# swiss-territorial-data-lab/proj-roadsurf

Measured on AMD Instinct MI355X. Metric: tiles_per_sec_512x512x3, higher is better.
Workload: dtype f16 hi + lo operand planes (22 significand bits, 3 MFMA products per product) / f32 accumulate; 1 GPU; Mask R-CNN R50-FPN inference, batch 16 of 512x512 3-band tiles per GPU (BASELINE configs[1]), 800x800 network input; seeded synthetic weights, saturated: 1000 proposals and 100 detections per tile; batch_per_gpu=16, lanes=2, lane_streams=independent, num_classes=2, weights=random

## Files before the change

### proj_roadsurf_amd/csrc/conv_wide1x1_split.hip

```cpp
#include "conv_tile.h"

namespace {

constexpr int PR = 32;
constexpr int KS = 8;
constexpr int SLICE = KS * PR * 128;
constexpr int LDS_BYTES = 2 * SLICE;

__device__ __forceinline__ float dot_term(float s, float v, float w, bool fused) {
  if (fused) return __builtin_fmaf(v, w, s);
  {
#pragma clang fp contract(off)
    const float m = v * w;
    return s + m;
  }
}

template <int NW, int NJ, int MODE>
__global__ __launch_bounds__(NW * 64, NW == 4 ? 2 : 1) void conv_wide1x1_split_kernel(const ConvParams p) {
  constexpr int BM = NW * NJ * 16;
  constexpr int NG = 32 / NW;
  constexpr int ST = MODE == 2 ? NJ : 4 * NJ;
  extern __shared__ __attribute__((aligned(16))) char smem[];
  const int tid = threadIdx.x, lane = tid & 63;
  const int wave = __builtin_amdgcn_readfirstlane(tid >> 6);
  const int M = conv_rows(p);
  const int ntiles = (M + BM - 1) / BM;
  const int q = blockIdx.x;
  if (q >= ntiles) return;
  const int m0 = xcd_tile(q, ntiles) * BM;
  const int rows = p.Cout * (MODE == 2 ? 4 : 1);
  const int npass = rows / PR;

  const int lrow = lane >> 3, lchk = lane & 7;
  const int rp = wave & 3, s0 = wave >> 2;
  const half_t* wsrc;
  {
    const int d = src_chunk(lchk, w_key(8 * rp + lrow, 8));
    wsrc = p.w + (long long)(rp * 16 + lrow) * p.Kpad + s0 * 32 + chunk_split(d, p.w_lo);
  }
  auto stage_piece = [&](int pass, int k) {
    const half_t* g = wsrc + (long long)((pass >> 1) * 64 + (pass & 1) * 8) * p.Kpad;
    char* base = smem + (pass & 1) * SLICE + (s0 * PR + rp * 8) * 128;
    glds16(g + k * (NW / 4) * 32, base + k * (NW / 4) * PR * 128);
  };

  const int fi = lane & 15, fq = lane >> 4, fkey = lane & 7;
  int w_off[2];
#pragma unroll
  for (int ii = 0; ii < 2; ++ii) w_off[ii] = frag_row(fi, ii, 8) * 128;
  const int ch_off = frag_off(fq, fkey, 0), cl_off = frag_off(fq, fkey, 1);

  half8 xh[KS][NJ], xl[KS][NJ];
  bool valid[NJ];
  long long opix[NJ];
  const float* wv[NJ];
  const bool full = m0 + (wave + 1) * NJ * 16 <= M;
#pragma unroll
  for (int j = 0; j < NJ; ++j) {
    const int m = m0 + (wave * NJ + j) * 16 + fi;
    valid[j] = m < M;
    const int mm = valid[j] ? m : M - 1;
    const Pix px = pix_of(mm, p.Wo, p.Ho);
    const int x = px.x, y = px.y, n = px.n;
    const half_t* xp = p.in + ((long long)(n * p.in_Hp + y + p.in_off) * p.in_Wp + x + p.in_off) * 256 + fq * 8;
#pragma unroll
    for (int s = 0; s < KS; ++s) { xh[s][j] = *(const half8*)(xp + s * 32); xl[s][j] = *(const half8*)(xp + p.in_lo + s * 32); }
    if (MODE == 2) {
      const int slot = p.dot_slot[n];
      wv[j] = p.dot_w + (long long)p.dot_cls[slot] * p.Cout;
      opix[j] = (long long)slot * (4 * p.Ho * p.Wo) + (long long)(2 * y) * (2 * p.Wo) + 2 * x;
    } else {
      wv[j] = nullptr;
      opix[j] = (long long)(n * p.out_Hp + y + p.out_pad) * p.out_Wp + x + p.out_pad;
    }
  }
  const bool has_res = MODE == 0 && p.res != nullptr;
  half8 rh[NJ], rl[NJ], qh[NJ], ql[NJ];
  auto load_res = [&](int pass, half8* h, half8* l) {
    const int c = (pass >> 1) * 64 + fq * 16 + (pass & 1) * 8;
#pragma unroll
    for (int j = 0; j < NJ; ++j) {
      const half_t* rp2 = p.res + opix[j] * p.out_Cs + c;
      h[j] = *(const half8*)rp2;
      l[j] = *(const half8*)(rp2 + p.res_lo);
    }
  };
#pragma unroll
  for (int j = 0; j < NJ; ++j) { rh[j] = half8{0, 0, 0, 0, 0, 0, 0, 0}; rl[j] = rh[j]; qh[j] = rh[j]; ql[j] = rh[j]; }
#pragma unroll
  for (int k = 0; k < NG; ++k) stage_piece(0, k);
  if (has_res) load_res(0, rh, rl);

#pragma unroll
  for (int s = 0; s < KS; ++s)
#pragma unroll
    for (int j = 0; j < NJ; ++j) asm volatile("" ::"v"(xh[s][j]), "v"(xl[s][j]));
  float sdot[NJ], gsum[NJ];
  half8 kh[MODE == 0 ? NJ : 1], kl[MODE == 0 ? NJ : 1];
#pragma unroll
  for (int j = 0; j < NJ; ++j) { sdot[j] = 0.f; gsum[j] = 0.f; }
  int pend = 0;
  auto run_pass = [&](const int pass, half8 (&ch)[NJ], half8 (&cl)[NJ], half8 (&nh)[NJ], half8 (&nl)[NJ]) __attribute__((always_inline)) {
    if (pend) asm volatile("s_waitcnt vmcnt(%0)" ::"n"(ST) : "memory");
    else asm volatile("s_waitcnt vmcnt(0)" ::: "memory");
    asm volatile("s_waitcnt lgkmcnt(0)" ::: "memory");
    __builtin_amdgcn_s_barrier();
    const bool more = pass + 1 < npass;
    if (more && has_res) load_res(pass + 1, nh, nl);
    const int crow = (pass >> 1) * 64 + fq * 16 + (pass & 1) * 8;
    const int g = MODE == 2 ? crow / p.Cout : 0, cb = crow - g * p.Cout;
    float bias[8], wsc[8];
    float dw[MODE == 2 ? NJ : 1][8];
    auto load_epi = [&]() {
#pragma unroll
      for (int ii = 0; ii < 2; ++ii) {
        const f32x4 b4 = *(const f32x4*)(p.bias + crow + ii * 4), s4 = *(const f32x4*)(p.wscale + crow + ii * 4);
#pragma unroll
        for (int r = 0; r < 4; ++r) { bias[ii * 4 + r] = b4[r]; wsc[ii * 4 + r] = s4[r]; }
      }
      if (MODE == 2) {
#pragma unroll
        for (int j = 0; j < NJ; ++j)
#pragma unroll
          for (int ii = 0; ii < 2; ++ii) {
            const f32x4 w4 = *(const f32x4*)(wv[j] + cb + ii * 4);
#pragma unroll
            for (int r = 0; r < 4; ++r) dw[j][ii * 4 + r] = w4[r];
          }
      }
    };
    __builtin_amdgcn_sched_barrier(0);
    const char* sb = smem + (pass & 1) * SLICE;
    f32x4 acc[2][NJ];
#pragma unroll
    for (int ii = 0; ii < 2; ++ii)
#pragma unroll
      for (int j = 0; j < NJ; ++j) acc[ii][j] = f32x4{0.f, 0.f, 0.f, 0.f};
    auto frag = [&](int s, int ii, int off) { return *(const half8*)(sb + s * (PR * 128) + w_off[ii] + off); };
    half8 wh[2], wl[2], nwh[2];
#pragma unroll
    for (int ii = 0; ii < 2; ++ii) { wh[ii] = frag(0, ii, ch_off); wl[ii] = frag(0, ii, cl_off); }
#pragma unroll
    for (int s = 0; s < KS; ++s) {
      if (s + 1 < KS) {
#pragma unroll
        for (int ii = 0; ii < 2; ++ii) nwh[ii] = frag(s + 1, ii, ch_off);
      }
      if (s == KS - 2) load_epi();
      if (more && 2 * s < NG) { stage_piece(pass + 1, 2 * s); stage_piece(pass + 1, 2 * s + 1); }
      __builtin_amdgcn_sched_barrier(0);
#pragma unroll
      for (int ii = 0; ii < 2; ++ii)
#pragma unroll
        for (int j = 0; j < NJ; ++j) acc[ii][j] = __builtin_amdgcn_mfma_f32_16x16x32_f16(wh[ii], xl[s][j], acc[ii][j], 0, 0, 0);
#pragma unroll
      for (int ii = 0; ii < 2; ++ii)
#pragma unroll
        for (int j = 0; j < NJ; ++j) acc[ii][j] = __builtin_amdgcn_mfma_f32_16x16x32_f16(wh[ii], xh[s][j], acc[ii][j], 0, 0, 0);
      __builtin_amdgcn_sched_barrier(0);
#pragma unroll
      for (int ii = 0; ii < 2; ++ii)
#pragma unroll
        for (int j = 0; j < NJ; ++j) acc[ii][j] = __builtin_amdgcn_mfma_f32_16x16x32_f16(wl[ii], xh[s][j], acc[ii][j], 0, 0, 0);
      __builtin_amdgcn_sched_barrier(0);
      if (s + 1 < KS) {
#pragma unroll
        for (int ii = 0; ii < 2; ++ii) { wl[ii] = frag(s + 1, ii, cl_off); wh[ii] = nwh[ii]; }
      }
    }

    if (MODE == 2) {
#pragma unroll
      for (int j = 0; j < NJ; ++j) {
        float v[8];
#pragma unroll
        for (int ii = 0; ii < 2; ++ii)
#pragma unroll
          for (int r = 0; r < 4; ++r) v[ii * 4 + r] = acc[ii][j][r] * wsc[ii * 4 + r] + bias[ii * 4 + r];
        if (p.relu) {
#pragma unroll
          for (int e = 0; e < 8; ++e) v[e] = v[e] > 0.f ? v[e] : 0.f;
        }
        float sd = sdot[j];
#pragma unroll
        for (int e = 0; e < 8; ++e) sd = dot_term(sd, v[e], dw[j][e], (pass & 1) == 0 && e < 4);
        sdot[j] = sd;
      }
      pend = 0;
      if (pass & 1) {
        const int blocks = p.Cout >> 6, k = (pass >> 1) % blocks;
#pragma unroll
        for (int j = 0; j < NJ; ++j) {
          float v0 = sdot[j];
          v0 += __shfl_xor(v0, 16);
          v0 += __shfl_xor(v0, 32);
          gsum[j] = k == 0 ? v0 : gsum[j] + v0;
          sdot[j] = 0.f;
        }
        if (k == blocks - 1) {
#pragma unroll
          for (int j = 0; j < NJ; ++j)
            if (fq == 0 && valid[j]) p.dot_out[opix[j] + (long long)(g >> 1) * (2 * p.Wo) + (g & 1)] = gsum[j];
          pend = full ? ST : 0;
        }
      }
    } else {
#pragma unroll
      for (int j = 0; j < NJ; ++j) {
        float v[8];
#pragma unroll
        for (int ii = 0; ii < 2; ++ii)
#pragma unroll
          for (int r = 0; r < 4; ++r) v[ii * 4 + r] = acc[ii][j][r] * wsc[ii * 4 + r] + bias[ii * 4 + r];
        if (has_res) {
#pragma unroll
          for (int e = 0; e < 8; ++e) v[e] += (float)ch[j][e] + (float)cl[j][e];
        }
        if (p.relu) {
#pragma unroll
          for (int e = 0; e < 8; ++e) v[e] = v[e] > 0.f ? v[e] : 0.f;
        }
        float scr = 0.f;
        half8 h, l;
#pragma unroll
        for (int e = 0; e < 8; ++e) {
          const float f = clamp_h16(v[e]);
          scr += __builtin_fabsf(f);
          const HiLo hl = split_round(f);
          h[e] = hl.h;
          l[e] = hl.l;
        }
        if (valid[j] && !(scr < 65504.f)) {
          unsigned c = 0;
#pragma unroll
          for (int e = 0; e < 8; ++e) c += rs_sat_bad(v[e]);
          rs_sat_flush(p.sat, c);
        }
        if ((pass & 1) == 0) {
          kh[j] = h; kl[j] = l;
        } else if (valid[j]) {
          half_t* op = (half_t*)p.out + opix[j] * p.out_Cs + crow - 8;
          *(half8*)op = kh[j];
          *(half8*)(op + 8) = h;
          *(half8*)(op + p.out_lo) = kl[j];
          *(half8*)(op + p.out_lo + 8) = l;
        }
      }
      pend = (pass & 1) && full ? ST : 0;
    }
  };
  for (int pass = 0; pass < npass; pass += 2) {
    run_pass(pass, rh, rl, qh, ql);
    run_pass(pass + 1, qh, ql, rh, rl);
  }
}

template <int NW, int NJ>
int launch_px(const ConvParams& p, hipStream_t stream) {
  const long long nblk = cdiv(p.M, NW * NJ * 16);
  RS_CHECK(nblk > 0 && nblk < (1ll << 31), RS_ERR_ARG, "conv_wide1x1_split: bad grid %lld", nblk);
  const void* k = p.mode == 2 ? (const void*)conv_wide1x1_split_kernel<NW, NJ, 2> : (const void*)conv_wide1x1_split_kernel<NW, NJ, 0>;
  static bool attr[2] = {false, false};
  const int ai = p.mode == 2 ? 1 : 0;
  if (!attr[ai]) {
    RS_HIP(hipFuncSetAttribute(k, hipFuncAttributeMaxDynamicSharedMemorySize, LDS_BYTES));
    attr[ai] = true;
  }
  ConvParams pc = p;
  void* args[] = {&pc};
  RS_HIP(hipLaunchKernel(k, dim3((unsigned)nblk), dim3(NW * 64), args, LDS_BYTES, stream));
  return RS_OK;
}

}

bool conv_wide1x1_split_ok(const ConvParams& p) {
  const int rows = p.Cout * (p.mode != 0 ? 4 : 1);
  return p.split && p.KH == 1 && p.KW == 1 && p.stride == 1 && p.Cin == 256 && p.in_Cs == 256 && p.Kpad >= 256 && !p.in2 && !p.up && !p.out_f32 &&
         !p.koff && !p.head_w && p.nseg == 0 && !p.down && !p.res32 && !p.mask && p.out_stride <= 1 && rows > 0 && rows % 64 == 0 &&
         (p.mode == 0 || (p.mode == 2 && p.Cout == 256)) &&
         p.Kpad % 8 == 0 && p.in_lo % 8 == 0 && p.w_lo % 8 == 0 &&
         (p.mode != 0 || (p.out_Cs % 8 == 0 && p.out_Cs >= rows && p.out_lo % 8 == 0 && p.res_lo % 8 == 0));
}

int launch_conv_wide1x1_split(const ConvParams& p, hipStream_t stream, int tile_px) {
  RS_CHECK(conv_wide1x1_split_ok(p), RS_ERR_UNSUPPORTED, "conv_wide1x1_split: takes split-operand 1x1 / stride 1 / Cin 256 layers with rows %% 64 == 0 (mode 0, or mode 2 with Cout 256)");
  RS_CHECK(p.M > 0 && p.in && p.w && p.bias && p.wscale && (!p.m_count || p.m_mul > 0), RS_ERR_ARG, "conv_wide1x1_split: null argument");
  if (p.mode == 2) RS_CHECK(p.dot_w && p.dot_cls && p.dot_slot && p.dot_out, RS_ERR_ARG, "conv_wide1x1_split: the fused mask predictor needs its pointers");
  else RS_CHECK(p.out, RS_ERR_ARG, "conv_wide1x1_split: null output");
  switch (tile_px) {
    case 64: return launch_px<4, 1>(p, stream);
    case 128: return launch_px<4, 2>(p, stream);
    case 256: return launch_px<8, 2>(p, stream);
    default: rs_set_error("conv_wide1x1_split: tile of %d pixels (64, 128 or 256)", tile_px); return RS_ERR_ARG;
  }
}
```

### proj_roadsurf_amd/csrc/ops.hip

```cpp
#include <string.h>

#include <vector>

#include "../../include/rs_engine.h"
#include "detect.h"
#include "polygon_pool.h"
#include "train.h"
#include "train_stats.h"
#include "val_ap.h"

namespace {

struct OpScratch {
  hipStream_t stream;
  void* held[2] = {nullptr, nullptr};
  int n = 0;
  explicit OpScratch(void* s) : stream((hipStream_t)s) {}
  OpScratch(const OpScratch&) = delete;
  OpScratch& operator=(const OpScratch&) = delete;
  int alloc(void** p, size_t bytes) {
    RS_CHECK(n < 2, RS_ERR_ARG, "OpScratch: more than two buffers");
    RS_HIP(hipMalloc(p, bytes));
    held[n++] = *p;
    return RS_OK;
  }
  hipError_t sync() const { return n ? hipStreamSynchronize(stream) : hipSuccess; }
  ~OpScratch() {
    (void)sync();
    for (int i = 0; i < n; ++i) (void)hipFree(held[i]);
  }
};

}

extern "C" {

__global__ void fdiv_kernel(const float* a, const float* b, float* out, long long n) {
  const long long i = (long long)blockIdx.x * 256 + threadIdx.x;
  if (i < n) out[i] = rs_fdiv(a[i], b[i]);
}
int rs_op_fdiv(const float* a, const float* b, float* out, int64_t n, void* stream) {
  RS_CHECK(a && b && out && n > 0, RS_ERR_ARG, "bad argument");
  hipLaunchKernelGGL(fdiv_kernel, dim3((unsigned)((n + 255) / 256)), dim3(256), 0, (hipStream_t)stream, a, b, out, (long long)n);
  RS_HIP(hipGetLastError());
  return RS_OK;
}

int rs_memcpy_d2h(void* dst, const void* src, size_t n) {
  RS_HIP(hipMemcpy(dst, src, n, hipMemcpyDeviceToHost));
  return RS_OK;
}
int rs_memcpy_h2d(void* dst, const void* src, size_t n) {
  RS_HIP(hipMemcpy(dst, src, n, hipMemcpyHostToDevice));
  return RS_OK;
}

int rs_op_conv_variant(int m, int cin, int k, int cout, int cin2, int deconv2x, int out_f32, int* stages_out) {
  ConvParams p;
  memset(&p, 0, sizeof p);
  p.M = m; p.Cin = cin; p.KH = p.KW = k; p.Cout = cout; p.mode = deconv2x ? 1 : 0; p.out_f32 = out_f32;
  p.stride = 1; p.in_Cs = cin; p.out_Cs = cout;
  p.Kpad = (k * k * (cin < 64 ? 8 : cin) + cin2 + 63) / 64 * 64;
  if (cin < 64 && k == 7) p.Kpad = 256;
  static const half_t dummy = (half_t)0;
  if (cin2 > 0) { p.in2 = &dummy; p.Cin2 = cin2; }
  const int v = conv_choose_variant(p, -1, 1);
  if (stages_out) *stages_out = p.stages;
  return cin < 64 ? 5 : v;
}

int rs_op_conv_variant_split(int m, int cin, int k, int stride, int cout, int cin2, int deconv_predict, int* stages_out) {
  ConvParams p;
  memset(&p, 0, sizeof p);
  p.M = m; p.Cin = cin; p.KH = p.KW = k; p.Cout = cout; p.mode = deconv_predict ? 2 : 0;
  p.stride = stride; p.in_Cs = cin; p.out_Cs = cout; p.split = 1;
  p.Kpad = (k * k * (cin < 64 ? 8 : cin) + cin2 + 63) / 64 * 64;
  if (cin < 64 && k == 7) p.Kpad = 256;
  static const half_t dummy = (half_t)0;
  if (cin2 > 0) { p.in2 = &dummy; p.Cin2 = cin2; }
  const int v = conv_choose_variant(p, -1, 1);
  if (stages_out) *stages_out = p.stages;
  return cin < 64 ? 5 : v;
}

static long long* g_conv_probe = nullptr;
static thread_local unsigned long long* g_op_sat = nullptr;
struct SplitArgs { long long in_lo, w_lo, out_lo, res_lo, up_lo; const float* wscale; };
static int op_conv2d(const void* in, const void* w, const float* bias, void* out, const void* residual, const void* upsample_add,
                     int n, int hi, int wi, int cin, int in_halo, int kh, int kw, int stride, int pad, int cout, int kpad,
                     int out_halo, int relu, int out_f32, int deconv2x, int variant, int use_glds, void* stream,
                     const void* in2, int h2, int w2, int cin2, int in2_halo, int stride2, const SplitArgs* sa = nullptr) {
  RS_CHECK(in && w && bias && out, RS_ERR_ARG, "null argument");
  RS_CHECK(in_halo >= pad, RS_ERR_ARG, "input halo %d < pad %d", in_halo, pad);
  const int ho = (hi + 2 * pad - kh) / stride + 1, wo = (wi + 2 * pad - kw) / stride + 1;
  ConvParams p;
  memset(&p, 0, sizeof p);
  p.in = (const half_t*)in; p.w = (const half_t*)w; p.bias = bias; p.out = out;
  p.res = (const half_t*)residual; p.up = (const half_t*)upsample_add;
  p.M = n * ho * wo; p.Ho = ho; p.Wo = wo;
  p.in_Hp = hi + 2 * in_halo; p.in_Wp = wi + 2 * in_halo; p.in_Cs = cin; p.in_off = in_halo - pad;
  p.stride = stride; p.KH = kh; p.KW = kw; p.Cin = cin; p.Kpad = kpad; p.Cout = cout;
  const int oh = deconv2x ? 2 * ho : ho, ow = deconv2x ? 2 * wo : wo;
  p.out_Hp = oh + 2 * out_halo; p.out_Wp = ow + 2 * out_halo; p.out_Cs = cout; p.out_pad = out_halo;
  if (upsample_add) { p.up_Hp = ho / 2 + 2 * out_halo; p.up_Wp = wo / 2 + 2 * out_halo; p.up_Cs = cout; p.up_pad = out_halo; }
  p.relu = relu; p.mode = deconv2x ? 1 : 0; p.out_f32 = out_f32;
  p.probe = g_conv_probe;
  p.sat = g_op_sat;
  if (sa) {
    RS_CHECK(sa->wscale && !in2, RS_ERR_ARG, "split-operand conv: row scales missing (or a second K source, which the operator does not take)");
    p.split = 1; p.in_lo = sa->in_lo; p.w_lo = sa->w_lo; p.out_lo = sa->out_lo; p.res_lo = sa->res_lo; p.up_lo = sa->up_lo; p.wscale = sa->wscale;
  }
  if (in2) {
    RS_CHECK(stride2 >= 1 && (ho - 1) * stride2 < h2 && (wo - 1) * stride2 < w2, RS_ERR_ARG, "second source geometry");
    p.in2 = (const half_t*)in2; p.in2_Hp = h2 + 2 * in2_halo; p.in2_Wp = w2 + 2 * in2_halo; p.in2_Cs = cin2;
    p.in2_off = in2_halo; p.stride2 = stride2; p.Cin2 = cin2;
  }
  OpScratch scratch(stream);
  if (cin < 64 && use_glds >= 0) {
    RS_CHECK(cin == 8, RS_ERR_UNSUPPORTED, "small-Cin path needs cin == 8");
    std::vector<int> koff(kpad / 8, 0);
    for (int t = 0; t < kh * kw && t < (int)koff.size(); ++t) koff[t] = ((t / kw) * p.in_Wp + (t % kw)) * cin;
    int* koff_dev = nullptr;
    { int rc = scratch.alloc((void**)&koff_dev, koff.size() * 4); if (rc) return rc; }
    RS_HIP(hipMemcpy(koff_dev, koff.data(), koff.size() * 4, hipMemcpyHostToDevice));
    p.koff = koff_dev;
  }
  return launch_conv(p, (hipStream_t)stream, variant, use_glds);
}

int rs_debug_set_conv_probe(void* buffer) { g_conv_probe = (long long*)buffer; return RS_OK; }
int rs_op_set_saturation_counter(void* dev_u64) { g_op_sat = (unsigned long long*)dev_u64; return RS_OK; }

int rs_op_conv2d(const void* in, const void* w, const float* bias, void* out, const void* residual, const void* upsample_add,
                 int n, int hi, int wi, int cin, int in_halo, int kh, int kw, int stride, int pad, int cout, int kpad,
                 int out_halo, int relu, int out_f32, int deconv2x, int variant, int use_glds, void* stream) {
  return op_conv2d(in, w, bias, out, residual, upsample_add, n, hi, wi, cin, in_halo, kh, kw, stride, pad, cout, kpad, out_halo,
                   relu, out_f32, deconv2x, variant, use_glds, stream, nullptr, 0, 0, 0, 0, 1);
}

int rs_op_conv2d_split(const void* in, int64_t in_lo, const void* w, int64_t w_lo, const float* wscale, const float* bias, void* out, int64_t out_lo,
                       const void* residual, int64_t res_lo, const void* upsample_add, int64_t up_lo,
                       int n, int hi, int wi, int cin, int in_halo, int kh, int kw, int stride, int pad, int cout, int kpad,
                       int out_halo, int relu, int out_f32, int deconv2x, int variant, void* stream) {
  SplitArgs sa = {in_lo, w_lo, out_lo, res_lo, up_lo, wscale};
  return op_conv2d(in, w, bias, out, residual, upsample_add, n, hi, wi, cin, in_halo, kh, kw, stride, pad, cout, kpad, out_halo,
                   relu, out_f32, deconv2x, variant, 1, stream, nullptr, 0, 0, 0, 0, 1, &sa);
}

int rs_op_deconv_predict_split(const void* in, int64_t in_lo, const void* w, int64_t w_lo, const float* wscale, const float* bias, const float* dot_w, int classes,
                               const int32_t* cls, const int32_t* slot, const int32_t* count_dev, float* logits, int entries, int side, int variant, void* stream) {
  RS_CHECK(in && w && wscale && bias && dot_w && cls && slot && logits && entries > 0 && side > 0 && classes > 0, RS_ERR_ARG, "deconv_predict_split: bad argument");
  ConvParams p;
  memset(&p, 0, sizeof p);
  p.in = (const half_t*)in; p.w = (const half_t*)w; p.bias = bias; p.wscale = wscale;
  p.split = 1; p.in_lo = in_lo; p.w_lo = w_lo;
  p.M = entries * side * side; p.Ho = side; p.Wo = side;
  p.in_Hp = side + 2; p.in_Wp = side + 2; p.in_Cs = 256; p.in_off = 1; p.stride = 1; p.KH = p.KW = 1; p.Cin = 256; p.Kpad = 256; p.Cout = 256;
  p.out_Hp = 2 * side; p.out_Wp = 2 * side; p.out_Cs = 256; p.relu = 1; p.mode = 2;
  p.m_count = count_dev; p.m_mul = side * side;
  p.dot_w = dot_w; p.dot_cls = cls; p.dot_slot = slot; p.dot_out = logits; p.dot_k = classes;
  return launch_conv(p, (hipStream_t)stream, variant, 1);
}

int rs_op_conv2d_dual(const void* in, const void* in2, const void* w, const float* bias, void* out,
                      int n, int hi, int wi, int cin, int in_halo, int kh, int kw, int stride, int pad,
                      int h2, int w2, int cin2, int in2_halo, int stride2,
                      int cout, int kpad, int out_halo, int relu, int variant, void* stream) {
  RS_CHECK(in2, RS_ERR_ARG, "null argument");
  return op_conv2d(in, w, bias, out, nullptr, nullptr, n, hi, wi, cin, in_halo, kh, kw, stride, pad, cout, kpad, out_halo,
                   relu, 0, 0, variant, 1, stream, in2, h2, w2, cin2, in2_halo, stride2);
}

int rs_op_bneck_tail(const void* t1, const void* w2, const float* b2, const void* w3p, const float* b3, const void* x, void* out,
                     const void* w1p, const float* b1, void* t1n, const void* x0, const void* wsc, int n, int h, int w, int width, void* stream) {
  RS_CHECK(t1 && w2 && b2 && w3p && b3 && out && n > 0 && h > 0 && w > 0, RS_ERR_ARG, "bad argument");
  RS_CHECK(width == 64 || width == 128, RS_ERR_UNSUPPORTED, "bneck_tail: bottleneck width %d (64 or 128)", width);
  BneckParams p;
  memset(&p, 0, sizeof p);
  p.t1 = (const half_t*)t1; p.w2 = (const half_t*)w2; p.b2 = b2; p.w3p = (const half_t*)w3p; p.b3 = b3; p.x = (const half_t*)x; p.out = (half_t*)out;
  p.w1p = (const half_t*)w1p; p.b1 = b1; p.t1n = (half_t*)t1n; p.x0 = (const half_t*)x0; p.wsc = (const half_t*)wsc;
  p.M = n * h * w; p.H = h; p.W = w; p.Hp = h + 2; p.Wp = w + 2; p.CB = width / 64;
  p.sat = g_op_sat;
  return launch_bneck_tail(p, (hipStream_t)stream);
}

int rs_op_bneck_tail_split(const void* t1, int64_t t1_lo, const void* w2, const float* s2, const float* b2, const void* w3p, const float* s3, const float* b3,
                           const void* x, int64_t x_lo, void* out, int64_t out_lo, const void* w1p, const float* s1, const float* b1, void* t1n, int64_t t1n_lo,
                           const void* x0, int64_t x0_lo, int n, int h, int w, int width, void* stream) {
  RS_CHECK(t1 && w2 && s2 && b2 && w3p && s3 && b3 && (x || x0) && out && n > 0 && h > 0 && w > 0, RS_ERR_ARG, "bad argument");
  RS_CHECK(width == 64 || width == 128, RS_ERR_UNSUPPORTED, "bneck_tail_split: bottleneck width %d (64 or 128)", width);
  BneckSplitParams p;
  memset(&p, 0, sizeof p);
  p.t1 = (const half_t*)t1; p.t1_lo = t1_lo;
  p.w2 = (const half_t*)w2; p.w2_lo = (long long)width * 9 * width; p.s2 = s2; p.b2 = b2;
  p.w3p = (const half_t*)w3p; p.w3_lo = 4ll * width * (width + (x0 ? 64 : 0)); p.s3 = s3; p.b3 = b3;
  p.x = (const half_t*)x; p.x_lo = x_lo; p.x0 = (const half_t*)x0; p.x0_lo = x0_lo; p.out = (half_t*)out; p.out_lo = out_lo;
  p.w1p = (const half_t*)w1p; p.w1_lo = 4ll * width * width; p.s1 = s1; p.b1 = b1; p.t1n = (half_t*)t1n; p.t1n_lo = t1n_lo;
  p.M = n * h * w; p.H = h; p.W = w; p.Hp = h + 2; p.Wp = w + 2; p.CB = width / 64;
  p.sat = g_op_sat;
  return launch_bneck_tail_split(p, (hipStream_t)stream);
}

int rs_op_mask_overlap(const uint8_t* det_masks, int n_det, const uint8_t* label_masks, int n_labels, int h, int w, int32_t* inter,
                       int32_t* label_area, void* stream) {
  return launch_mask_overlap(det_masks, n_det, label_masks, n_labels, h, w, inter, label_area, (hipStream_t)stream);
}


int rs_op_rasterize_canvas(const double* polys, const int64_t* poly_off, const int32_t* poly_len, const int32_t* inst_first, int n_inst,
                           int side, uint8_t* out) {
  RS_CHECK(inst_first && n_inst >= 0 && (out || n_inst == 0), RS_ERR_ARG, "rasterize_canvas: null table");
  RS_CHECK(side >= 1 && side <= CR_MAX_SIDE, RS_ERR_ARG, "rasterize_canvas: side %d outside [1, %d]", side, CR_MAX_SIDE);
  MtLayout L;
  { int rc = mt_measure(polys, poly_off, poly_len, inst_first, n_inst, 0, &L); if (rc) return rc; }
  RS_CHECK(L.n_doubles <= (size_t)MT_MAX_DOUBLES, RS_ERR_UNSUPPORTED, "rasterize_canvas: more than %d doubles of polygons", MT_MAX_DOUBLES);
  if (n_inst == 0) return RS_OK;
  std::vector<uint8_t> host(L.bytes);
  const int32_t zero = 0;
  mt_pack(host.data(), L, polys, poly_off, poly_len, inst_first, &zero);
  const size_t bytes = (size_t)n_inst * side * ((side + 7) / 8);
  OpScratch scratch(nullptr);
  uint8_t *pool = nullptr, *m = nullptr;
  { int rc = scratch.alloc((void**)&pool, L.bytes); if (rc) return rc; }
  { int rc = scratch.alloc((void**)&m, bytes); if (rc) return rc; }
  RS_HIP(hipMemcpy(pool, host.data(), L.bytes, hipMemcpyHostToDevice));
  CanvasRasterParams q;
  memset(&q, 0, sizeof q);
  q.inst_first = (const int*)(pool + L.o_inst); q.poly_off = (const int*)(pool + L.o_off); q.poly_len = (const int*)(pool + L.o_len);
  q.polys = (const double*)(pool + L.o_xy); q.out = m; q.n_inst = n_inst; q.side = side;
  { int rc = launch_canvas_raster(q, nullptr); if (rc) return rc; }
  RS_HIP(hipMemcpy(out, m, bytes, hipMemcpyDeviceToHost));
  return RS_OK;
}

int rs_op_mask_pair_counts(const uint8_t* det_masks, const int32_t* det_count, int n_tiles, int slots, const uint8_t* gt_masks,
                           const int32_t* tile_first, int gt_cap, int side, int32_t* inter, int32_t* det_area, int32_t* gt_area, void* stream) {
  RS_CHECK(det_masks && det_count && tile_first && inter && det_area && gt_area, RS_ERR_ARG, "mask_pair_counts: null buffer");
  RS_CHECK(side >= 1 && side <= CR_MAX_SIDE, RS_ERR_ARG, "mask_pair_counts: side %d outside [1, %d]", side, CR_MAX_SIDE);
  RS_CHECK(n_tiles >= 1 && slots >= 1 && gt_cap >= 1, RS_ERR_ARG, "mask_pair_counts: %d tiles, %d slots, %d ground truths per tile", n_tiles, slots, gt_cap);
  PairCountParams q;
  memset(&q, 0, sizeof q);
  q.det_masks = det_masks; q.det_count = det_count; q.gt_masks = gt_masks; q.tile_first = tile_first;
  q.inter = inter; q.det_area = det_area; q.gt_area = gt_area; q.n = n_tiles; q.D = slots; q.g_cap = gt_cap;
  q.bytes = (long long)side * ((side + 7) / 8);
  return launch_mask_pair_counts(q, (hipStream_t)stream);
}

int rs_op_conv2d_dgrad(const void* dy, const void* w_t, void* dx, const void* res, const float* res32, const void* mask,
                       const void* down, int n, int hi, int wi, int cin, int ho, int wo, int cout, int kh, int kw, int stride,
                       int pad, int kpad, int halo, int variant, void* stream) {
  RS_CHECK(dy && w_t && dx, RS_ERR_ARG, "null argument");
  RS_CHECK(stride == 1 || (kh == 1 && kw == 1), RS_ERR_UNSUPPORTED, "dgrad: stride %d needs a 1x1 kernel (STRIDE_IN_1X1)", stride);
  RS_CHECK(halo >= kh - 1 - pad && halo >= 0 && kh == kw, RS_ERR_ARG, "dgrad: halo %d too small", halo);
  ConvParams p;
  memset(&p, 0, sizeof p);
  const int pad_t = kh - 1 - pad;
  const int oh = stride == 1 ? ho + 2 * pad_t - kh + 1 : ho, ow = stride == 1 ? wo + 2 * pad_t - kw + 1 : wo;
  RS_CHECK(stride == 1 ? (oh == hi && ow == wi) : ((ho - 1) * stride < hi && (wo - 1) * stride < wi), RS_ERR_ARG, "dgrad: geometry");
  OpScratch scratch(stream);
  void* zero_bias = nullptr;
  { int rc = scratch.alloc(&zero_bias, (size_t)cin * 4 + 256); if (rc) return rc; }
  RS_HIP(hipMemsetAsync(zero_bias, 0, (size_t)cin * 4 + 256, (hipStream_t)stream));
  p.in = (const half_t*)dy; p.w = (const half_t*)w_t; p.bias = (const float*)zero_bias; p.out = dx;
  p.res = (const half_t*)res; p.res32 = res32; p.mask = (const half_t*)mask; p.down = (const half_t*)down;
  p.M = n * oh * ow; p.Ho = oh; p.Wo = ow;
  p.in_Hp = ho + 2 * halo; p.in_Wp = wo + 2 * halo; p.in_Cs = cout; p.in_off = halo - pad_t;
  p.stride = 1; p.KH = kh; p.KW = kw; p.Cin = cout; p.Kpad = kpad; p.Cout = cin;
  p.out_Hp = hi + 2 * halo; p.out_Wp = wi + 2 * halo; p.out_Cs = cin; p.out_pad = halo;
  p.out_stride = stride;
  if (down) { p.down_Hp = 2 * hi + 2 * halo; p.down_Wp = 2 * wi + 2 * halo; p.down_Cs = cin; p.down_pad = halo; }
  return launch_conv(p, (hipStream_t)stream, variant, 1);
}

int rs_op_conv2d_dgrad_split(const void* dy, const void* w_t, void* dx, const void* res, const float* res32, const void* mask,
                             const void* down, int n, int hi, int wi, int cin, int ho, int wo, int cout, int kh, int kw, int stride,
                             int pad, int kpad, int halo, int variant, const int32_t* count_dev, void* stream) {
  RS_CHECK(dy && w_t && dx, RS_ERR_ARG, "rs_op_conv2d_dgrad_split: null operand");
  RS_CHECK(n >= 1, RS_ERR_ARG, "rs_op_conv2d_dgrad_split: n %d", n);
  RS_CHECK(cout >= 64 && cout % 64 == 0, RS_ERR_ARG, "rs_op_conv2d_dgrad_split: cout %d (the K side) must be a multiple of 64", cout);
  RS_CHECK(stride == 1 || (stride > 1 && kh == 1 && kw == 1), RS_ERR_UNSUPPORTED, "rs_op_conv2d_dgrad_split: stride %d needs a 1x1 kernel", stride);
  RS_CHECK(kh == kw && kh >= 1 && pad >= 0 && halo >= 0 && halo >= kh - 1 - pad, RS_ERR_ARG, "rs_op_conv2d_dgrad_split: halo %d below k - 1 - pad = %d", halo, kh - 1 - pad);
  RS_CHECK(hi >= 1 && wi >= 1 && ho >= 1 && wo >= 1 && cin >= 16 && cin % 16 == 0 && kpad >= kh * kw * cout && kpad % 64 == 0, RS_ERR_ARG,
           "rs_op_conv2d_dgrad_split: geometry (cin %d must be a multiple of 16, kpad %d at least kh * kw * cout and a multiple of 64)", cin, kpad);
  RS_CHECK(conv_dgrad_split_serves(cin, cout, kh, kw, stride), RS_ERR_UNSUPPORTED, "rs_op_conv2d_dgrad_split: shape not served");
  const int pad_t = kh - 1 - pad;
  const int oh = stride == 1 ? ho + 2 * pad_t - kh + 1 : ho, ow = stride == 1 ? wo + 2 * pad_t - kw + 1 : wo;
  RS_CHECK(stride == 1 ? (oh == hi && ow == wi) : ((ho - 1) * stride < hi && (wo - 1) * stride < wi), RS_ERR_ARG, "rs_op_conv2d_dgrad_split: geometry");
  ConvParams p;
  memset(&p, 0, sizeof p);
  p.out = dx; p.res = (const half_t*)res; p.res32 = res32; p.mask = (const half_t*)mask; p.down = (const half_t*)down;
  p.M = n * oh * ow; p.Ho = oh; p.Wo = ow;
  p.in_Hp = ho + 2 * halo; p.in_Wp = wo + 2 * halo; p.in_Cs = cout; p.in_off = halo - pad_t;
  p.stride = 1; p.KH = kh; p.KW = kw; p.Cin = cout; p.Kpad = kpad; p.Cout = cin;
  p.out_Hp = hi + 2 * halo; p.out_Wp = wi + 2 * halo; p.out_Cs = cin; p.out_pad = halo;
  p.out_stride = stride;
  if (down) { p.down_Hp = 2 * hi + 2 * halo; p.down_Wp = 2 * wi + 2 * halo; p.down_Cs = cin; p.down_pad = halo; }
  if (count_dev) { p.m_count = count_dev; p.m_mul = oh * ow; }
  const long long cap = (long long)n * p.in_Hp * p.in_Wp * cout;
  const size_t b_dy = (dgrad_split_scratch_bytes(cap) + 255) & ~(size_t)255, b_w = ((size_t)cin * kpad * 4 + 255) & ~(size_t)255;
  hipStream_t s = (hipStream_t)stream;
  OpScratch scratch(stream);
  char* buf = nullptr;
  { int rc = scratch.alloc((void**)&buf, b_dy + b_w + (size_t)cin * 4); if (rc) return rc; }
  p.in = (const half_t*)dy;
  { int rc = launch_dgrad_split_planes(p, buf, cap, s); if (rc) return rc; }
  SplitRowsDesc d = {(const float*)w_t, (half_t*)(buf + b_dy), (float*)(buf + b_dy + b_w), cin, kpad, 0u};
  { int rc = launch_split_rows(d, s); if (rc) return rc; }
  p.split = 1; p.dy_amax = (const unsigned*)buf;
  p.in = (const half_t*)(buf + WGS_HEAD_BYTES); p.in_lo = cap;
  p.w = d.planes; p.w_lo = (long long)cin * kpad; p.wscale = d.inv;
  return launch_conv(p, s, variant, 1);
}
int rs_op_conv2d_dgrad_split_serves(int cin, int cout, int kh, int stride) {
  return conv_dgrad_split_serves(cin, cout, kh, kh, stride) ? 1 : 0;
}
int rs_op_conv2d_fwd_split(const void* x, const void* w, const float* bias, void* y, const void* res, const void* up, int n, int hi, int wi,
                           int cin, int in_halo, int kh, int kw, int stride, int pad, int cout, int kpad, int out_halo, int relu, int variant,
                           const int32_t* count_dev, void* stream) {
  RS_CHECK(x && w && bias && y, RS_ERR_ARG, "rs_op_conv2d_fwd_split: null operand");
  RS_CHECK(n >= 1, RS_ERR_ARG, "rs_op_conv2d_fwd_split: n %d", n);
  RS_CHECK(cin >= 64 && cin % 64 == 0, RS_ERR_ARG, "rs_op_conv2d_fwd_split: cin %d (the K side) must be a multiple of 64", cin);
  RS_CHECK(cout >= 16 && cout % 16 == 0, RS_ERR_ARG, "rs_op_conv2d_fwd_split: cout %d (the rows) must be a multiple of 16", cout);
  RS_CHECK(kh == kw && kh >= 1 && stride >= 1 && pad >= 0 && out_halo >= 0 && in_halo >= pad, RS_ERR_ARG, "rs_op_conv2d_fwd_split: halo %d below the pad %d (or a kernel that is not square, stride %d)", in_halo, pad, stride);
  RS_CHECK(hi >= 1 && wi >= 1 && hi + 2 * pad >= kh && wi + 2 * pad >= kw && kpad >= kh * kw * cin && kpad % 64 == 0, RS_ERR_ARG,
           "rs_op_conv2d_fwd_split: geometry (%d x %d input, %dx%d kernel, kpad %d at least kh * kw * cin and a multiple of 64)", hi, wi, kh, kw, kpad);
  RS_CHECK(conv_fwd_split_serves(cout, cin, kh, kw, stride), RS_ERR_UNSUPPORTED, "rs_op_conv2d_fwd_split: shape not served");
  const int ho = (hi + 2 * pad - kh) / stride + 1, wo = (wi + 2 * pad - kw) / stride + 1;
  ConvParams p;
  memset(&p, 0, sizeof p);
  p.bias = bias; p.out = y; p.res = (const half_t*)res; p.up = (const half_t*)up;
  p.M = n * ho * wo; p.Ho = ho; p.Wo = wo;
  p.in_Hp = hi + 2 * in_halo; p.in_Wp = wi + 2 * in_halo; p.in_Cs = cin; p.in_off = in_halo - pad;
  p.stride = stride; p.KH = kh; p.KW = kw; p.Cin = cin; p.Kpad = kpad; p.Cout = cout;
  p.out_Hp = ho + 2 * out_halo; p.out_Wp = wo + 2 * out_halo; p.out_Cs = cout; p.out_pad = out_halo;
  if (up) { p.up_Hp = (ho + 1) / 2 + 2 * out_halo; p.up_Wp = (wo + 1) / 2 + 2 * out_halo; p.up_Cs = cout; p.up_pad = out_halo; }
  p.relu = relu ? 1 : 0;
  if (count_dev) { p.m_count = count_dev; p.m_mul = ho * wo; }
  const long long cap = (long long)n * p.in_Hp * p.in_Wp * cin;
  const size_t b_x = (dgrad_split_scratch_bytes(cap) + 255) & ~(size_t)255, b_w = ((size_t)cout * kpad * 4 + 255) & ~(size_t)255;
  hipStream_t s = (hipStream_t)stream;
  OpScratch scratch(stream);
  char* buf = nullptr;
  { int rc = scratch.alloc((void**)&buf, b_x + b_w + (size_t)cout * 4); if (rc) return rc; }
  p.in = (const half_t*)x;
  { int rc = launch_fwd_split_planes(p, buf, cap, s); if (rc) return rc; }
  SplitRowsDesc d = {(const float*)w, (half_t*)(buf + b_x), (float*)(buf + b_x + b_w), cout, kpad, 0u};
  { int rc = launch_split_rows(d, s); if (rc) return rc; }
  p.split = 1; p.x_amax = (const unsigned*)buf;
  p.in = (const half_t*)(buf + WGS_HEAD_BYTES); p.in_lo = cap;
  p.w = d.planes; p.w_lo = (long long)cout * kpad; p.wscale = d.inv;
  return launch_conv(p, s, variant, 1);
}
int rs_op_conv2d_fwd_split_serves(int cin, int cout, int k, int stride) {
  return conv_fwd_split_serves(cout, cin, k, k, stride) ? 1 : 0;
}
int rs_op_split_rows(const float* w, int rows, int k, void* planes, float* inv_scale, void* stream) {
  RS_CHECK(w && planes && inv_scale && rows >= 1 && k >= 1, RS_ERR_ARG, "rs_op_split_rows: bad argument");
  SplitRowsDesc d = {w, (half_t*)planes, inv_scale, rows, k, 0u};
  return launch_split_rows(d, (hipStream_t)stream);
}

static int op_conv2d_wgrad(const void* dy, const void* x, float* grad, const float* scale, int n, int hi, int wi, int cin, int in_halo,
                           int kh, int kw, int stride, int pad, int cout, int kpad, int dy_halo, int splits, void* stream, int f32);
int rs_op_conv2d_wgrad(const void* dy, const void* x, float* grad, const float* scale, int n, int hi, int wi, int cin, int in_halo,
                       int kh, int kw, int stride, int pad, int cout, int kpad, int dy_halo, int splits, void* stream) {
  return op_conv2d_wgrad(dy, x, grad, scale, n, hi, wi, cin, in_halo, kh, kw, stride, pad, cout, kpad, dy_halo, splits, stream, 0);
}
int rs_op_conv2d_wgrad_f32(const void* dy, const void* x, float* grad, const float* scale, int n, int hi, int wi, int cin, int in_halo,
                           int kh, int kw, int stride, int pad, int cout, int kpad, int dy_halo, int splits, void* stream) {
  return op_conv2d_wgrad(dy, x, grad, scale, n, hi, wi, cin, in_halo, kh, kw, stride, pad, cout, kpad, dy_halo, splits, stream, 1);
}
int rs_op_conv2d_wgrad_split(const void* dy, const void* x, float* grad, const float* scale, int n, int hi, int wi, int cin, int in_halo,
                             int kh, int kw, int stride, int pad, int cout, int kpad, int dy_halo, int splits, void* stream) {
  RS_CHECK(dy && x && grad, RS_ERR_ARG, "rs_op_conv2d_wgrad_split: null operand");
  RS_CHECK(n >= 1 && hi >= 1 && wi >= 1 && kh >= 1 && kw >= 1 && stride >= 1 && pad >= 0 && in_halo >= pad && dy_halo >= 0 && hi + 2 * pad >= kh &&
           wi + 2 * pad >= kw, RS_ERR_ARG, "rs_op_conv2d_wgrad_split: geometry (%d x %d x %d input, %dx%d kernel, stride %d, pad %d, halos %d / %d)",
           n, hi, wi, kh, kw, stride, pad, in_halo, dy_halo);
  RS_CHECK(cin >= 64 && cin % 64 == 0 && cout >= 1 && cout % 4 == 0 && kpad == kh * kw * cin, RS_ERR_ARG,
           "rs_op_conv2d_wgrad_split: cin %d must be a multiple of 64, cout %d of 4, and kpad %d = kh * kw * cin", cin, cout, kpad);
  return op_conv2d_wgrad(dy, x, grad, scale, n, hi, wi, cin, in_halo, kh, kw, stride, pad, cout, kpad, dy_halo, splits, stream, 2);
}
int rs_op_conv2d_wgrad_split_serves(int cin, int cout) {
  WgradParams p;
  memset(&p, 0, sizeof p);
  p.f32 = 1; p.Cin = cin; p.in_Cs = cin; p.Cout = cout; p.dy_Cs = cout;
  return cin >= 64 && cout >= 1 && wgrad_split_serves(p) ? 1 : 0;
}
static int op_conv2d_wgrad(const void* dy, const void* x, float* grad, const float* scale, int n, int hi, int wi, int cin, int in_halo,
                           int kh, int kw, int stride, int pad, int cout, int kpad, int dy_halo, int splits, void* stream, int f32) {
  RS_CHECK(dy && x && grad, RS_ERR_ARG, "null argument");
  RS_CHECK(in_halo >= pad, RS_ERR_ARG, "input halo %d < pad %d", in_halo, pad);
  const int ho = (hi + 2 * pad - kh) / stride + 1, wo = (wi + 2 * pad - kw) / stride + 1;
  WgradParams p;
  memset(&p, 0, sizeof p);
  p.dy = (const half_t*)dy; p.x = (const half_t*)x; p.grad = grad; p.scale = scale;
  p.M = n * ho * wo; p.Ho = ho; p.Wo = wo;
  p.dy_Hp = ho + 2 * dy_halo; p.dy_Wp = wo + 2 * dy_halo; p.dy_Cs = cout; p.dy_pad = dy_halo;
  p.in_Hp = hi + 2 * in_halo; p.in_Wp = wi + 2 * in_halo; p.in_Cs = cin; p.in_off = in_halo - pad;
  p.stride = stride; p.KH = kh; p.KW = kw; p.Cin = cin; p.Cout = cout; p.Kpad = kpad;
  p.f32 = f32 ? 1 : 0;
  p.split_ops = f32 == 2;
  p.splits = splits > 0 ? splits : wgrad_splits(p);
  hipStream_t s = (hipStream_t)stream;
  OpScratch scratch(stream);
  void *partial = nullptr, *zeros = nullptr;
  { int rc = scratch.alloc(&partial, (size_t)p.splits * cout * kpad * 4); if (rc) return rc; }
  size_t planes = 0;
  if (p.split_ops) {
    p.split_dy_cap = (long long)n * p.dy_Hp * p.dy_Wp * p.dy_Cs;
    p.split_x_cap = (long long)n * p.in_Hp * p.in_Wp * p.in_Cs;
    planes = (wgrad_split_scratch_bytes(p.split_dy_cap, p.split_x_cap) + 255) & ~(size_t)255;
  }
  { int rc = scratch.alloc(&zeros, planes + (size_t)cout * 2 + 256); if (rc) return rc; }
  if (p.split_ops) {
    p.split_scratch = zeros;
    RS_HIP(hipMemsetAsync(zeros, 0, WGS_HEAD_BYTES, s));
    zeros = (char*)zeros + planes;
  }
  RS_HIP(hipMemsetAsync(zeros, 0, (size_t)cout * 2 + 256, s));
  RS_HIP(hipMemsetAsync(partial, 0, (size_t)p.splits * cout * kpad * 4, s));
  p.partial = (float*)partial; p.zeros = (const half_t*)zeros;
  return launch_conv_wgrad(p, s);
}

int rs_op_maxpool3x3s2_bwd(const void* x, const void* dq, void* dx, int n, int hc, int wc, int c, int x_halo, int q_halo, int f32, void* stream) {
  RS_CHECK(x && dq && dx, RS_ERR_ARG, "rs_op_maxpool3x3s2_bwd: null operand");
  RS_CHECK(n >= 1 && hc >= 1 && wc >= 1 && c >= 1 && x_halo >= 0 && q_halo >= 0, RS_ERR_ARG,
           "rs_op_maxpool3x3s2_bwd: geometry (%d x %d x %d x %d, halos %d / %d)", n, hc, wc, c, x_halo, q_halo);
  PoolBwdParams p;
  memset(&p, 0, sizeof p);
  p.x = x; p.dq = dq; p.dx = dx;
  p.N = n; p.Hc = hc; p.Wc = wc; p.Hq = (hc - 1) / 2 + 1; p.Wq = (wc - 1) / 2 + 1; p.C = c; p.x_halo = x_halo; p.q_halo = q_halo;
  p.f32 = f32 ? 1 : 0;
  return launch_maxpool3x3s2_bwd(p, (hipStream_t)stream);
}
static int op_stem_wgrad(const void* dy, const void* x0, float* grad, const float* scale, int n, int hc, int wc, int cin, int dy_halo,
                         int x_halo, int splits, void* stream, int f32) {
  RS_CHECK(dy && x0 && grad, RS_ERR_ARG, "rs_op_stem_wgrad: null operand");
  RS_CHECK(n >= 1 && hc >= 1 && wc >= 1 && (long long)n * hc * wc < (1ll << 31) - 8 && 4 / wc < hc, RS_ERR_ARG, "rs_op_stem_wgrad: %d x %d x %d pixels", n, hc, wc);
  RS_CHECK(cin >= 1 && cin <= 4 && dy_halo >= 0 && x_halo >= 3, RS_ERR_ARG, "rs_op_stem_wgrad: %d input channels of 4, halos %d / %d (input: at least 3)", cin, dy_halo, x_halo);
  RS_CHECK(splits <= RS_STEM_WGRAD_MAX_SPLITS, RS_ERR_ARG, "rs_op_stem_wgrad: %d splits, at most %d", splits, RS_STEM_WGRAD_MAX_SPLITS);
  StemWgradParams p;
  memset(&p, 0, sizeof p);
  p.dy = dy; p.x0 = x0; p.scale = scale; p.grad = grad;
  p.N = n; p.Hc = hc; p.Wc = wc; p.dy_halo = dy_halo; p.x_halo = x_halo; p.cin = cin;
  p.splits = splits > 0 ? splits : stem_wgrad_splits((long long)n * hc * wc);
  p.f32 = f32;
  OpScratch scratch(stream);
  { int rc = scratch.alloc((void**)&p.partial, (size_t)p.splits * 64 * RS_STEM_KPAD * 4); if (rc) return rc; }
  return launch_stem_wgrad(p, (hipStream_t)stream);
}
int rs_op_stem_wgrad(const void* dy, const void* x0, float* grad, const float* scale, int n, int hc, int wc, int cin, int dy_halo,
                     int x_halo, int splits, void* stream) {
  return op_stem_wgrad(dy, x0, grad, scale, n, hc, wc, cin, dy_halo, x_halo, splits, stream, 0);
}
int rs_op_stem_wgrad_f32(const void* dy, const void* x0, float* grad, const float* scale, int n, int hc, int wc, int cin, int dy_halo,
                         int x_halo, int splits, void* stream) {
  return op_stem_wgrad(dy, x0, grad, scale, n, hc, wc, cin, dy_halo, x_halo, splits, stream, 1);
}

int rs_op_nms(const float* boxes, const int32_t* counts, const uint8_t* valid, uint8_t* keep, int segments, int cap,
              float thresh, void* stream) {
  RS_CHECK(boxes && counts && keep && segments > 0, RS_ERR_ARG, "bad argument");
// ... 308 lines not shown
```

Baseline: 948.3 tiles/s.

## Stage bias/scale/dot tables in LDS and restructure pass barrier into publish step

New measurement: 953.5 tiles/s, median of 6. No clear change (+0.5%).

```diff
diff --git a/proj_roadsurf_amd/csrc/conv_wide1x1_split.hip b/proj_roadsurf_amd/csrc/conv_wide1x1_split.hip
--- a/proj_roadsurf_amd/csrc/conv_wide1x1_split.hip
+++ b/proj_roadsurf_amd/csrc/conv_wide1x1_split.hip
@@ -5,7 +5,12 @@
 constexpr int PR = 32;
 constexpr int KS = 8;
 constexpr int SLICE = KS * PR * 128;
-constexpr int LDS_BYTES = 2 * SLICE;
+constexpr int TAB_ROWS = 1024;
+constexpr int DOT_COUT = 256;
+constexpr int DOT_CAP = 4;
+constexpr int DOT_PITCH = 256 + 4;
+constexpr int TAB_OFF = 2 * SLICE, DOT_OFF = TAB_OFF + 2 * TAB_ROWS * 4;
+constexpr int lds_bytes(int mode, bool table) { return !table ? TAB_OFF : (mode == 2 ? DOT_OFF + DOT_CAP * DOT_PITCH * 4 : DOT_OFF); }
 
 __device__ __forceinline__ float dot_term(float s, float v, float w, bool fused) {
   if (fused) return __builtin_fmaf(v, w, s);
@@ -16,11 +21,10 @@
   }
 }
 
-template <int NW, int NJ, int MODE>
+template <int NW, int NJ, int MODE, bool TABLE>
 __global__ __launch_bounds__(NW * 64, NW == 4 ? 2 : 1) void conv_wide1x1_split_kernel(const ConvParams p) {
   constexpr int BM = NW * NJ * 16;
   constexpr int NG = 32 / NW;
-  constexpr int ST = MODE == 2 ? NJ : 4 * NJ;
   extern __shared__ __attribute__((aligned(16))) char smem[];
   const int tid = threadIdx.x, lane = tid & 63;
   const int wave = __builtin_amdgcn_readfirstlane(tid >> 6);
@@ -55,7 +59,7 @@
   bool valid[NJ];
   long long opix[NJ];
   const float* wv[NJ];
-  const bool full = m0 + (wave + 1) * NJ * 16 <= M;
+  const int ent0 = MODE == 2 ? m0 / (p.Ho * p.Wo) : 0;
 #pragma unroll
   for (int j = 0; j < NJ; ++j) {
     const int m = m0 + (wave * NJ + j) * 16 + fi;
@@ -68,7 +72,8 @@
     for (int s = 0; s < KS; ++s) { xh[s][j] = *(const half8*)(xp + s * 32); xl[s][j] = *(const half8*)(xp + p.in_lo + s * 32); }
     if (MODE == 2) {
       const int slot = p.dot_slot[n];
-      wv[j] = p.dot_w + (long long)p.dot_cls[slot] * p.Cout;
+      if (TABLE) wv[j] = (const float*)(smem + DOT_OFF) + min(n - ent0, DOT_CAP - 1) * DOT_PITCH;
+      else wv[j] = p.dot_w + (long long)p.dot_cls[slot] * p.Cout;
       opix[j] = (long long)slot * (4 * p.Ho * p.Wo) + (long long)(2 * y) * (2 * p.Wo) + 2 * x;
     } else {
       wv[j] = nullptr;
@@ -76,7 +81,6 @@
     }
   }
   const bool has_res = MODE == 0 && p.res != nullptr;
-  half8 rh[NJ], rl[NJ], qh[NJ], ql[NJ];
   auto load_res = [&](int pass, half8* h, half8* l) {
     const int c = (pass >> 1) * 64 + fq * 16 + (pass & 1) * 8;
 #pragma unroll
@@ -87,10 +91,24 @@
     }
   };
 #pragma unroll
-  for (int j = 0; j < NJ; ++j) { rh[j] = half8{0, 0, 0, 0, 0, 0, 0, 0}; rl[j] = rh[j]; qh[j] = rh[j]; ql[j] = rh[j]; }
-#pragma unroll
   for (int k = 0; k < NG; ++k) stage_piece(0, k);
-  if (has_res) load_res(0, rh, rl);
+  if (TABLE) {
+    float* tb = (float*)(smem + TAB_OFF);
+    for (int i = tid * 4; i < rows; i += NW * 64 * 4) {
+      *(f32x4*)(tb + i) = *(const f32x4*)(p.bias + i);
+      *(f32x4*)(tb + TAB_ROWS + i) = *(const f32x4*)(p.wscale + i);
+    }
+    if (MODE == 2) {
+      const int last = (min(m0 + BM, M) - 1) / (p.Ho * p.Wo);
+      const int ne = min(last - ent0 + 1, DOT_CAP);
+      float* dt = (float*)(smem + DOT_OFF);
+      for (int i = tid; i < ne * 64; i += NW * 64) {
+        const int e = i >> 6, c = (i & 63) * 4;
+        const float* row = p.dot_w + (long long)p.dot_cls[p.dot_slot[ent0 + e]] * p.Cout;
+        *(f32x4*)(dt + e * DOT_PITCH + c) = *(const f32x4*)(row + c);
+      }
+    }
+  }
 
 #pragma unroll
   for (int s = 0; s < KS; ++s)
@@ -100,22 +118,53 @@
   half8 kh[MODE == 0 ? NJ : 1], kl[MODE == 0 ? NJ : 1];
 #pragma unroll
   for (int j = 0; j < NJ; ++j) { sdot[j] = 0.f; gsum[j] = 0.f; }
-  int pend = 0;
-  auto run_pass = [&](const int pass, half8 (&ch)[NJ], half8 (&cl)[NJ], half8 (&nh)[NJ], half8 (&nl)[NJ]) __attribute__((always_inline)) {
-    if (pend) asm volatile("s_waitcnt vmcnt(%0)" ::"n"(ST) : "memory");
-    else asm volatile("s_waitcnt vmcnt(0)" ::: "memory");
+#ifdef RS_WIDE1X1_PHASES
+  unsigned long long ph_t = __builtin_amdgcn_s_memtime(), ph_loop = 0, ph_vm = 0, ph_lds = 0, ph_bar = 0, ph_epi = 0;
+  const unsigned long long ph_entry = ph_t;
+#define RS_PH(acc) { const unsigned long long t_ = __builtin_amdgcn_s_memtime(); acc += t_ - ph_t; ph_t = t_; }
+#else
+#define RS_PH(acc)
+#endif
+  auto publish = [&]() {
+    RS_PH(ph_loop)
+    asm volatile("s_waitcnt vmcnt(0)" ::: "memory");
+    RS_PH(ph_vm)
     asm volatile("s_waitcnt lgkmcnt(0)" ::: "memory");
+    RS_PH(ph_lds)
     __builtin_amdgcn_s_barrier();
+    asm volatile("" ::: "memory");
+    RS_PH(ph_bar)
+  };
+  auto frag = [&](const char* sb, int s, int ii, int off) { return *(const half8*)(sb + s * (PR * 128) + w_off[ii] + off); };
+  half8 wh[2], wl[2];
+  auto first_frags = [&](int pass) {
+    const char* sb = smem + (pass & 1) * SLICE;
+#pragma unroll
+    for (int ii = 0; ii < 2; ++ii) { wh[ii] = frag(sb, 0, ii, ch_off); wl[ii] = frag(sb, 0, ii, cl_off); }
+  };
+  publish();
+  first_frags(0);
+#ifdef RS_WIDE1X1_PHASES
+  const unsigned long long ph_pro = ph_t - ph_entry;
+  ph_loop = ph_vm = ph_lds = ph_bar = 0;
+#endif
+  auto run_pass = [&](const int pass) __attribute__((always_inline)) {
     const bool more = pass + 1 < npass;
-    if (more && has_res) load_res(pass + 1, nh, nl);
-    const int crow = (pass >> 1) * 64 + fq * 16 + (pass & 1) * 8;
-    const int g = MODE == 2 ? crow / p.Cout : 0, cb = crow - g * p.Cout;
+    half8 ch[NJ], cl[NJ];
+#pragma unroll
+    for (int j = 0; j < NJ; ++j) { ch[j] = half8{0, 0, 0, 0, 0, 0, 0, 0}; cl[j] = ch[j]; }
+    if (has_res) load_res(pass, ch, cl);
+    const int blk = (pass >> 1) * 64;
+    const int crow = blk + fq * 16 + (pass & 1) * 8;
+    const int g = MODE == 2 ? blk / DOT_COUT : 0, cb = crow - g * DOT_COUT;
     float bias[8], wsc[8];
     float dw[MODE == 2 ? NJ : 1][8];
     auto load_epi = [&]() {
+      const float* bsrc = TABLE ? (const float*)(smem + TAB_OFF) : p.bias;
+      const float* ssrc = TABLE ? (const float*)(smem + TAB_OFF) + TAB_ROWS : p.wscale;
 #pragma unroll
       for (int ii = 0; ii < 2; ++ii) {
-        const f32x4 b4 = *(const f32x4*)(p.bias + crow + ii * 4), s4 = *(const f32x4*)(p.wscale + crow + ii * 4);
+        const f32x4 b4 = *(const f32x4*)(bsrc + crow + ii * 4), s4 = *(const f32x4*)(ssrc + crow + ii * 4);
 #pragma unroll
         for (int r = 0; r < 4; ++r) { bias[ii * 4 + r] = b4[r]; wsc[ii * 4 + r] = s4[r]; }
       }
@@ -137,15 +186,12 @@
     for (int ii = 0; ii < 2; ++ii)
 #pragma unroll
       for (int j = 0; j < NJ; ++j) acc[ii][j] = f32x4{0.f, 0.f, 0.f, 0.f};
-    auto frag = [&](int s, int ii, int off) { return *(const half8*)(sb + s * (PR * 128) + w_off[ii] + off); };
-    half8 wh[2], wl[2], nwh[2];
-#pragma unroll
-    for (int ii = 0; ii < 2; ++ii) { wh[ii] = frag(0, ii, ch_off); wl[ii] = frag(0, ii, cl_off); }
+    half8 nwh[2];
 #pragma unroll
     for (int s = 0; s < KS; ++s) {
       if (s + 1 < KS) {
 #pragma unroll
-        for (int ii = 0; ii < 2; ++ii) nwh[ii] = frag(s + 1, ii, ch_off);
+        for (int ii = 0; ii < 2; ++ii) nwh[ii] = frag(sb, s + 1, ii, ch_off);
       }
       if (s == KS - 2) load_epi();
       if (more && 2 * s < NG) { stage_piece(pass + 1, 2 * s); stage_piece(pass + 1, 2 * s + 1); }
@@ -166,8 +212,14 @@
       __builtin_amdgcn_sched_barrier(0);
       if (s + 1 < KS) {
 #pragma unroll
-        for (int ii = 0; ii < 2; ++ii) { wl[ii] = frag(s + 1, ii, cl_off); wh[ii] = nwh[ii]; }
-      }
+        for (int ii = 0; ii < 2; ++ii) { wl[ii] = frag(sb, s + 1, ii, cl_off); wh[ii] = nwh[ii]; }
+      }
+    }
+
+    if (more) {
+      publish();
+      first_frags(pass + 1);
+      __builtin_amdgcn_sched_barrier(0);
     }
 
     if (MODE == 2) {
@@ -187,9 +239,9 @@
         for (int e = 0; e < 8; ++e) sd = dot_term(sd, v[e], dw[j][e], (pass & 1) == 0 && e < 4);
         sdot[j] = sd;
       }
-      pend = 0;
       if (pass & 1) {
-        const int blocks = p.Cout >> 6, k = (pass >> 1) % blocks;
+        constexpr int blocks = DOT_COUT >> 6;
+        const int k = (pass >> 1) % blocks;
 #pragma unroll
         for (int j = 0; j < NJ; ++j) {
           float v0 = sdot[j];
@@ -202,7 +254,6 @@
 #pragma unroll
           for (int j = 0; j < NJ; ++j)
             if (fq == 0 && valid[j]) p.dot_out[opix[j] + (long long)(g >> 1) * (2 * p.Wo) + (g & 1)] = gsum[j];
-          pend = full ? ST : 0;
         }
       }
     } else {
@@ -247,29 +298,42 @@
           *(half8*)(op + p.out_lo + 8) = l;
         }
       }
-      pend = (pass & 1) && full ? ST : 0;
     }
   };
   for (int pass = 0; pass < npass; pass += 2) {
-    run_pass(pass, rh, rl, qh, ql);
-    run_pass(pass + 1, qh, ql, rh, rl);
-  }
+    run_pass(pass);
+    RS_PH(ph_epi)
+    run_pass(pass + 1);
+    RS_PH(ph_epi)
+  }
+#ifdef RS_WIDE1X1_PHASES
+  if (p.probe && lane == 0) {
+    long long* o = p.probe + ((long long)q * 8 + wave) * 8;
+    o[0] = (long long)ph_loop; o[1] = (long long)ph_vm; o[2] = (long long)ph_lds; o[3] = (long long)ph_bar; o[4] = (long long)ph_epi; o[5] = npass;
+    o[6] = (long long)ph_pro; o[7] = (long long)(ph_t - ph_entry);
+  }
+#endif
+#undef RS_PH
 }
 
 template <int NW, int NJ>
 int launch_px(const ConvParams& p, hipStream_t stream) {
   const long long nblk = cdiv(p.M, NW * NJ * 16);
   RS_CHECK(nblk > 0 && nblk < (1ll << 31), RS_ERR_ARG, "conv_wide1x1_split: bad grid %lld", nblk);
-  const void* k = p.mode == 2 ? (const void*)conv_wide1x1_split_kernel<NW, NJ, 2> : (const void*)conv_wide1x1_split_kernel<NW, NJ, 0>;
-  static bool attr[2] = {false, false};
-  const int ai = p.mode == 2 ? 1 : 0;
+  const int mode = p.mode == 2 ? 2 : 0, rows = p.Cout * (mode == 2 ? 4 : 1);
+  const bool table = rows <= TAB_ROWS && (mode == 0 || (NW * NJ * 16) / (p.Ho * p.Wo) + 2 <= DOT_CAP);
+  const void* k = mode == 2 ? (table ? (const void*)conv_wide1x1_split_kernel<NW, NJ, 2, true> : (const void*)conv_wide1x1_split_kernel<NW, NJ, 2, false>)
+                            : (table ? (const void*)conv_wide1x1_split_kernel<NW, NJ, 0, true> : (const void*)conv_wide1x1_split_kernel<NW, NJ, 0, false>);
+  const int lds = lds_bytes(mode, table);
+  static bool attr[4] = {false, false, false, false};
+  const int ai = (mode == 2 ? 2 : 0) + (table ? 1 : 0);
   if (!attr[ai]) {
-    RS_HIP(hipFuncSetAttribute(k, hipFuncAttributeMaxDynamicSharedMemorySize, LDS_BYTES));
+    RS_HIP(hipFuncSetAttribute(k, hipFuncAttributeMaxDynamicSharedMemorySize, lds));
     attr[ai] = true;
   }
   ConvParams pc = p;
   void* args[] = {&pc};
-  RS_HIP(hipLaunchKernel(k, dim3((unsigned)nblk), dim3(NW * 64), args, LDS_BYTES, stream));
+  RS_HIP(hipLaunchKernel(k, dim3((unsigned)nblk), dim3(NW * 64), args, lds, stream));
   return RS_OK;
 }
 
@@ -279,7 +343,7 @@
   const int rows = p.Cout * (p.mode != 0 ? 4 : 1);
   return p.split && p.KH == 1 && p.KW == 1 && p.stride == 1 && p.Cin == 256 && p.in_Cs == 256 && p.Kpad >= 256 && !p.in2 && !p.up && !p.out_f32 &&
          !p.koff && !p.head_w && p.nseg == 0 && !p.down && !p.res32 && !p.mask && p.out_stride <= 1 && rows > 0 && rows % 64 == 0 &&
-         (p.mode == 0 || (p.mode == 2 && p.Cout == 256)) &&
+         (p.mode == 0 || (p.mode == 2 && p.Cout == DOT_COUT)) &&
          p.Kpad % 8 == 0 && p.in_lo % 8 == 0 && p.w_lo % 8 == 0 &&
          (p.mode != 0 || (p.out_Cs % 8 == 0 && p.out_Cs >= rows && p.out_lo % 8 == 0 && p.res_lo % 8 == 0));
 }
@@ -287,7 +351,7 @@
 int launch_conv_wide1x1_split(const ConvParams& p, hipStream_t stream, int tile_px) {
   RS_CHECK(conv_wide1x1_split_ok(p), RS_ERR_UNSUPPORTED, "conv_wide1x1_split: takes split-operand 1x1 / stride 1 / Cin 256 layers with rows %% 64 == 0 (mode 0, or mode 2 with Cout 256)");
   RS_CHECK(p.M > 0 && p.in && p.w && p.bias && p.wscale && (!p.m_count || p.m_mul > 0), RS_ERR_ARG, "conv_wide1x1_split: null argument");
-  if (p.mode == 2) RS_CHECK(p.dot_w && p.dot_cls && p.dot_slot && p.dot_out, RS_ERR_ARG, "conv_wide1x1_split: the fused mask predictor needs its pointers");
+  if (p.mode == 2) RS_CHECK(p.dot_w && p.dot_cls && p.dot_slot && p.dot_out && p.Ho > 0 && p.Wo > 0, RS_ERR_ARG, "conv_wide1x1_split: the fused mask predictor needs its pointers");
   else RS_CHECK(p.out, RS_ERR_ARG, "conv_wide1x1_split: null output");
   switch (tile_px) {
     case 64: return launch_px<4, 1>(p, stream);
diff --git a/proj_roadsurf_amd/csrc/ops.hip b/proj_roadsurf_amd/csrc/ops.hip
--- a/proj_roadsurf_amd/csrc/ops.hip
+++ b/proj_roadsurf_amd/csrc/ops.hip
@@ -159,6 +159,7 @@
   p.out_Hp = 2 * side; p.out_Wp = 2 * side; p.out_Cs = 256; p.relu = 1; p.mode = 2;
   p.m_count = count_dev; p.m_mul = side * side;
   p.dot_w = dot_w; p.dot_cls = cls; p.dot_slot = slot; p.dot_out = logits; p.dot_k = classes;
+  p.probe = g_conv_probe;
   return launch_conv(p, (hipStream_t)stream, variant, 1);
 }
 
```
